# uberkk/ImageCompressionLearnedLiftingandLearnedTreeBasedModels

Measured on AMD Instinct MI355X. Metric: Mpixels/sec (lifting DWT + entropy-model fwd) at 512x512 RGB, higher is better.
Workload: dtype f32 storage, f16x3 arithmetic (3 fp16 MFMA products per fp32 MAC, fp32 accumulate)

## Files before the change

### imagecompressionlearnedliftingandlearnedtreebasedmodels_amd/csrc/conv_f16x3.hip

```cpp
#include "common.h"
#include "split_f16.h"
#include "lifting_f16.h"
#include "plc_fold.h"
#include <string.h>
#include <type_traits>

namespace lldwt {

constexpr int F3_CK = 32;
constexpr int F3_TH = 8, F3_TW = 32;
constexpr int F3_IH = F3_TH + 2, F3_IW = F3_TW + 2, F3_NPX = F3_IH * F3_IW;
constexpr int F3_PITCH = F3_CK * 2 + 16;
constexpr int F3_PART = F3_NPX * F3_PITCH;
constexpr int F3_BUF = 2 * F3_PART;
constexpr int F3_LDS = 2 * F3_BUF + 64;
constexpr int F3_OCB = 128;
constexpr int F3_STEP_BYTES = 2048;
constexpr int F3_CHUNK_BYTES = 9 * 2 * F3_STEP_BYTES;
constexpr int F3_HDR = 256;
constexpr int F3_NTASK = F3_NPX * (F3_CK / 8);
constexpr int F3_R = (F3_NTASK + 255) / 256;

constexpr int F1_HDR = 2048;
constexpr int F1_CHUNK_BYTES = 2 * F3_STEP_BYTES;
// ... 113 lines not shown
    for (int o = 32; o > 0; o >>= 1) {
        mw = fmaxf(mw, __shfl_xor(mw, o, 64));
        ml1 = fmaxf(ml1, __shfl_xor(ml1, o, 64));
        mb = fmaxf(mb, __shfl_xor(mb, o, 64));
    }
    if ((tid & 63) == 0) { red[0][tid >> 6] = mw; red[1][tid >> 6] = ml1; red[2][tid >> 6] = mb; }
    __syncthreads();
    const float amw = fmaxf(fmaxf(red[0][0], red[0][1]), fmaxf(red[0][2], red[0][3]));
    const float sw1 = pow2_scale<15>(amw);
    if (tid == 0) {
        hdr[0] = sw1;
        hdr[1] = fmaxf(fmaxf(red[1][0], red[1][1]), fmaxf(red[1][2], red[1][3]));
        hdr[2] = fmaxf(fmaxf(red[2][0], red[2][1]), fmaxf(red[2][2], red[2][3]));
    }
    const int nch = (cmid + F3_CK - 1) / F3_CK;
    for (int i = tid; i < nch * F3_CK; i += 256) hdr[16 + i] = i < cmid ? bp[i] : 0.f;
    _Float16* fr = reinterpret_cast<_Float16*>(pp + F1_HDR);
    for (int i = tid; i < nch * 2 * 512; i += 256) {
        const int j = i & 7, lane = (i >> 3) & 63, ks = (i >> 9) & 1, chunk = i >> 10;
        const int c = chunk * F3_CK + (lane & 31), k = 16 * ks + 8 * (lane >> 5) + j;
        float v = 0.f;
        if (c < cmid && k < 27) v = wp[c * 27 + k] * sw1;
        const _Float16 hi = (_Float16)v;
        fr[(chunk * 2 + ks) * 1024 + lane * 8 + j] = hi;
        fr[(chunk * 2 + ks) * 1024 + 512 + lane * 8 + j] = (_Float16)(v - (float)hi);
        reinterpret_cast<__bf16*>(pp + F1_HDR + (int64_t)nch * F1_CHUNK_BYTES)[(chunk * 2 + ks) * 512 + lane * 8 + j] = (__bf16)v;
    }
    _Float16* f16 = reinterpret_cast<_Float16*>(pp + f1_w16_off(cmid));
    for (int i = tid; i < w3_nch(cmid) * 512; i += 256) {
        const int j = i & 7, lane = (i >> 3) & 63, chunk = i >> 9;
        const int c = chunk * W3_CK + (lane & 15), k = 8 * (lane >> 4) + j;
        float v = 0.f;
        if (c < cmid && k < 27) v = wp[c * 27 + k] * sw1;
        const _Float16 hi = (_Float16)v;
        f16[chunk * 1024 + lane * 8 + j] = hi;
        f16[chunk * 1024 + 512 + lane * 8 + j] = (_Float16)(v - (float)hi);
    }
}

struct F3Args {
    const float* x;
    float* y;
    const uint8_t* packed;
    const float* bias;
    const float* slots;
    const _Float16* x16;
    const float* xscale;
    const float* parent;
    const uint8_t* packed1;
    int64_t plane_bytes1;
    int cin, cout, act, batch, h, w, tiles_x, nch;
    int64_t plane_bytes;
    unsigned long long* stamps;
};
#define F3_STAMP(i)                                                                                                     \
    if (a.stamps && lane == 0)                                                                                          \
        a.stamps[((((int64_t)blockIdx.z * gridDim.y + blockIdx.y) * gridDim.x + blockIdx.x) * 4 + wave) * 16 + (i)] =   \
            (i) >= 14 ? __builtin_amdgcn_s_memrealtime() : __builtin_amdgcn_s_memtime();

template <int MODE, int PREC = 0, bool S16 = false>
__global__ __launch_bounds__(256) __attribute__((amdgpu_waves_per_eu(1, 1))) void k_conv3_f16x3(F3Args a) {
    constexpr bool IN16 = MODE == 1, FUSED = MODE == 2;
    static_assert(PREC == 0 || FUSED, "the one-product modes exist for the fused pair (eval path)");
    constexpr int SB = PREC == 2 ? F3_STEP_BYTES / 2 : F3_STEP_BYTES;
    extern __shared__ __attribute__((aligned(16))) uint8_t lds[];
    const int tid = threadIdx.x, lane = tid & 63, wave = tid >> 6;
    const int64_t z = blockIdx.z;
    const int plane = (int)(z / a.batch);
    const int ocb = blockIdx.y;
    const int ty = blockIdx.x / a.tiles_x, tx = blockIdx.x - ty * a.tiles_x;
    const int y0 = ty * F3_TH, x0 = tx * F3_TW;
    const int h = a.h, w = a.w;
    const int64_t hw = (int64_t)h * w;

    F3_STAMP(0)
    F3_STAMP(14)
    float sx = 1.f;
    if constexpr (IN16) {
        sx = a.xscale[plane];
    } else if constexpr (FUSED) {
    } else {
        float amax = a.slots[plane * 64 + lane];
#pragma unroll
        for (int o = 32; o > 0; o >>= 1) amax = fmaxf(amax, __shfl_xor(amax, o, 64));
        sx = pow2_scale<15>(amax);
    }
    const uint8_t* pp = a.packed + (int64_t)plane * a.plane_bytes;
    const float sw = *reinterpret_cast<const float*>(pp);
    float out_scale = (1.f / sx) * (1.f / sw);

    unsigned pix[F3_R];
    int icg8[F3_R];
    int woff[F3_R];
    bool inimg[F3_R];
#pragma unroll
    for (int r = 0; r < F3_R; ++r) {
        const int task = tid + r * 256;
        const bool live = task < F3_NTASK;
        const int icg = live ? task / F3_NPX : 0, p = live ? task - icg * F3_NPX : 0;
        const int ly = p / F3_IW, lx = p - ly * F3_IW;
        const int gy = y0 - 1 + ly, gx = x0 - 1 + lx;
        const bool in = live && gy >= 0 && gy < h && gx >= 0 && gx < w;
        inimg[r] = in;
        icg8[r] = icg * 8;
        woff[r] = p * F3_PITCH + icg * 16;
        pix[r] = in ? (IN16 ? 2u : 4u) * (unsigned)(gy * w + gx) : 0u;
// ... 545 lines not shown
__device__ __forceinline__ void wino_u(const float* g, double (&u)[4]) {
    const double g0 = g[0], g1 = g[1], g2 = g[2];
    u[0] = g0; u[1] = (g0 + g1 + g2) * 0.5; u[2] = (g0 - g1 + g2) * 0.5; u[3] = g2;
}

__global__ void k_f3w_umax(const float* __restrict__ w, int64_t nrows, uint8_t* __restrict__ packed, int64_t plane_bytes, int64_t woff) {
    const int plane = blockIdx.y;
    float m = 0.f;
    for (int64_t i = blockIdx.x * (int64_t)blockDim.x + threadIdx.x; i < nrows; i += (int64_t)gridDim.x * blockDim.x) {
        double u[4];
        wino_u(w + ((int64_t)plane * nrows + i) * 3, u);
        for (int k = 0; k < 4; ++k) m = fmaxf(m, fabsf((float)u[k]));
    }
#pragma unroll
    for (int o = 32; o > 0; o >>= 1) m = fmaxf(m, __shfl_down(m, o, 64));
    float* hdr = reinterpret_cast<float*>(packed + (int64_t)plane * plane_bytes + woff);
    if ((threadIdx.x & 63) == 0 && m > 0.f) atomicMax(reinterpret_cast<int*>(hdr + 1), __float_as_int(m));
}

__global__ void k_f3w_pack(const float* __restrict__ w, uint8_t* __restrict__ packed, int cin, int cout, int64_t plane_bytes, int64_t woff) {
    const int plane = blockIdx.y;
    uint8_t* pp = packed + (int64_t)plane * plane_bytes + woff;
    float* hdr = reinterpret_cast<float*>(pp);
    const double su = pow2_scale<15>(hdr[1]);
    const int nch = w3_nch(cin), nocb = (cout + F3_OCB - 1) / F3_OCB;
    const int64_t n = (int64_t)nocb * 4 * nch * W3_NST * 64 * 8;
    const float* wp = w + (int64_t)plane * cout * cin * 9;
    _Float16* out = reinterpret_cast<_Float16*>(pp + F3_HDR);
    for (int64_t i = blockIdx.x * (int64_t)blockDim.x + threadIdx.x; i < n; i += (int64_t)gridDim.x * blockDim.x) {
        int64_t r = i;
        const int j = (int)(r % 8); r /= 8;
        const int lane = (int)(r % 64); r /= 64;
        const int st = (int)(r % W3_NST); r /= W3_NST;
        const int chunk = (int)(r % nch); r /= nch;
        const int wv = (int)(r % 4); r /= 4;
        const int ocb = (int)r;
        const int oc = ocb * F3_OCB + wv * 32 + (lane & 31), ic = chunk * W3_CK + 8 * (lane >> 5) + j;
        const int dy = st >> 2, xi = st & 3;
        float v = 0.f;
        if (oc < cout && ic < cin) {
            double u[4];
            wino_u(wp + ((int64_t)oc * cin + ic) * 9 + dy * 3, u);
            v = (float)(u[xi] * su);
        }
        const _Float16 hi = (_Float16)v;
        const int64_t step = ((int64_t)(ocb * 4 + wv) * nch + chunk) * W3_NST + st;
        out[step * 1024 + lane * 8 + j] = hi;
        out[step * 1024 + 512 + lane * 8 + j] = (_Float16)(v - (float)hi);
    }
    if (blockIdx.x == 0 && threadIdx.x == 0) hdr[0] = (float)su;
}

template <bool EARLIER>
__global__ __launch_bounds__(256) __attribute__((amdgpu_waves_per_eu(1, 1))) void k_plc_wino(F3Args a) {
    extern __shared__ __attribute__((aligned(16))) uint8_t lds[];
    const int tid = threadIdx.x, lane = tid & 63, wave = tid >> 6;
    const int64_t z = blockIdx.z;
    const int plane = (int)(z / a.batch);
    const int nocb = (a.cout + F3_OCB - 1) / F3_OCB;
    const int npass = (!EARLIER && gridDim.y == 1) ? nocb : 1;
    int ocb = blockIdx.y;
#define W3_STAMP(i)                                                                                                     \
    if (a.stamps && lane == 0)                                                                                          \
        a.stamps[((((int64_t)blockIdx.z * nocb + ocb) * gridDim.x + blockIdx.x) * 4 + wave) * 16 + (i)] =               \
            (i) >= 14 ? __builtin_amdgcn_s_memrealtime() : __builtin_amdgcn_s_memtime();
    const int ty = blockIdx.x / a.tiles_x, tx = blockIdx.x - ty * a.tiles_x;
    const int y0 = ty * F3_TH, x0 = tx * F3_TW;
    const int h = a.h, w = a.w;
    const int64_t hw = (int64_t)h * w;

    W3_STAMP(0)
    W3_STAMP(14)
    const uint8_t* pp = a.packed + (int64_t)plane * a.plane_bytes + f3_wino_off(a.cin, a.cout);
    const float su = *reinterpret_cast<const float*>(pp);
    const uint8_t* pk1 = a.packed1 + (int64_t)plane * a.plane_bytes1;
    const float* h1 = reinterpret_cast<const float*>(pk1);
    const float* bias1 = h1 + 16;
    const int hp = h >> 1, wp_ = w >> 1;
    const float* par = a.parent + z * 3 * (int64_t)hp * wp_;
    static_assert(F1_PP <= 512, "two patch values per thread");
    float pv[2] = {0.f, 0.f};
    if constexpr (!EARLIER) {
#pragma unroll
        for (int k = 0; k < 2; ++k) {
            const int i = min(tid + 256 * k, F1_PP - 1);
            const int ci = i / 108, rem = i - ci * 108, r = rem / 18, c = rem - r * 18;
            const int Yp = (y0 >> 1) - 1 + r, Xp = (x0 >> 1) - 1 + c;
            pv[k] = par[(int64_t)ci * hp * wp_ + min(max(Yp, 0), hp - 1) * wp_ + min(max(Xp, 0), wp_ - 1)];
        }
    }
    const uint8_t* wbase = pp + F3_HDR + ((int64_t)(ocb * 4 + wave) * a.nch) * (W3_NST * F3_STEP_BYTES) + lane * 16;
    half8 ah[W3_RING], al[W3_RING];
#pragma unroll
    for (int i = 0; i < W3_RING - 1; ++i) {
        ah[i] = *reinterpret_cast<const half8*>(wbase + i * F3_STEP_BYTES);
        al[i] = *reinterpret_cast<const half8*>(wbase + i * F3_STEP_BYTES + 1024);
    }
    half8 w1h, w1l;
    f4_t b1r, b1v;
#define W3_FUSED_LOAD(C1)                                                                                             \
    {                                                                                                                 \
        const uint8_t* w1_ = pk1 + f1_w16_off(a.cin) + (int64_t)((C1) / W3_CK) * F3_STEP_BYTES + lane * 16;           \
        w1h = *reinterpret_cast<const half8*>(w1_);                                                                   \
        w1l = *reinterpret_cast<const half8*>(w1_ + 1024);                                                            \
        b1r = *reinterpret_cast<const f4_t*>(bias1 + (C1) + 4 * (lane >> 4));                                        \
    }
    W3_FUSED_LOAD(0)
    float bias2 = 0.f, bias2n = 0.f;
#define W3_BIAS_LOAD(DST, OCB)                                                                                        \
    {                                                                                                                 \
        const int oc_ = (OCB) * F3_OCB + tid;                                                                         \
        if (tid < F3_OCB && a.bias && oc_ < a.cout) DST = a.bias[plane * a.cout + oc_];                               \
    }
    if constexpr (!EARLIER) {
        W3_BIAS_LOAD(bias2, ocb)
        if (npass > 1) W3_BIAS_LOAD(bias2n, ocb + 1)
    }

    float* PP = reinterpret_cast<float*>(lds + W3_PP);
    float amax = 0.f;
#pragma unroll
    for (int i = tid; i < F1_PP; i += 256) {
        const int ci = i / 108, rem = i - ci * 108, r = rem / 18, c = rem - r * 18;
        const int Yp = (y0 >> 1) - 1 + r, Xp = (x0 >> 1) - 1 + c;
        const bool in = Yp >= 0 && Yp < hp && Xp >= 0 && Xp < wp_;
        const float v = EARLIER ? par[(int64_t)ci * hp * wp_ + min(max(Yp, 0), hp - 1) * wp_ + min(max(Xp, 0), wp_ - 1)] : pv[i >> 8];
        const float vz = in ? v : 0.f;
        PP[i] = vz;
        amax = fmaxf(amax, fabsf(vz));
    }
#pragma unroll
    for (int o = 32; o > 0; o >>= 1) amax = fmaxf(amax, __shfl_xor(amax, o, 64));
    float* red = reinterpret_cast<float*>(lds + W3_DUMP + 32);
    if (lane == 0) red[wave] = amax;
    __syncthreads();
    amax = fmaxf(fmaxf(red[0], red[1]), fmaxf(red[2], red[3]));
    const float s_p = pow2_scale<15>(amax);
    const float sx = 0.5f * pow2_scale<15>(amax * h1[1] + h1[2]);
    const float out_scale = (1.f / sx) * (1.f / su);
    const float inv1sx = (1.f / s_p) * (1.f / h1[0]) * sx;
    W3_STAMP(12)
    if constexpr (EARLIER) {
    for (int px = tid; px < F3_NPX; px += 256) {
        const int ly = px / F3_IW, lx = px - ly * F3_IW;
        uint8_t* dst = lds + W3_COL + ((lx & 1) * (F3_IH * 17) + ly * 17 + (lx >> 1)) * W3_COLP;
#pragma unroll
        for (int g = 0; g < 4; ++g) {
            float v8[8];
#pragma unroll
            for (int j = 0; j < 8; ++j) {
                const int k = 8 * g + j, q = k < 27 ? k : 26;
                const int dy = (q % 9) / 3, dx = q % 3;
                v8[j] = PP[(q / 9) * 108 + ((ly + dy) >> 1) * 18 + ((lx + dx) >> 1)] * s_p;
            }
            half8 ch_, cl_;
            split8v(v8, ch_, cl_);
            *reinterpret_cast<half8*>(dst + g * 16) = ch_;
            *reinterpret_cast<half8*>(dst + 64 + g * 16) = cl_;
        }
    }
    } else {
        switch (__builtin_amdgcn_readfirstlane(wave)) {
            case 0: w3_im2col_group<0>(lds, PP, s_p, lane); break;
            case 1: w3_im2col_group<1>(lds, PP, s_p, lane); break;
            case 2: w3_im2col_group<2>(lds, PP, s_p, lane); break;
            default: w3_im2col_group<3>(lds, PP, s_p, lane); break;
        }
    }

    const int p = lane & 15, g = lane >> 4;
    int colw[3], vw[3];
    unsigned pinm = 0;
// ... 5 lines not shown
        const int rr = live ? r : 0;
        colw[B] = W3_COL + (rr * 17 + p) * W3_COLP + g * 16;
        vw[B] = live ? ((rr * 4) * 16 + p) * 32 + (((g >> 1) ^ (p >> 3)) * 16) + (g & 1) * 8 : -1;
        const int gy = y0 - 1 + r;
#pragma unroll
        for (int s = 0; s < 4; ++s) {
            const int gx = x0 - 1 + 2 * p + s;
            pin[B][s] = live && gy >= 0 && gy < h && gx >= 0 && gx < w;
            if (pin[B][s]) pinm |= 1u << (4 * B + s);
        }
    }
    const int en = p < 6 ? p : 0, er = wave + 4 * (en >> 1);
    const bool elive = p < 6 && er < F3_IH;
    const int cole = W3_COL + (((en & 1) * F3_IH + (elive ? er : 0)) * 17 + 16) * W3_COLP + g * 16;
    const int pine = (elive && y0 - 1 + er >= 0 && y0 - 1 + er < h && x0 + 31 + (en & 1) < w) ? -1 : 0;
    half8 c1h[4], c1l[4];
    f4_t t1[4];
    float d1[4][4];
#define W3_ROW_READ(B)                                                                                                \
    {                                                                                                                 \
        _Pragma("unroll") for (int s = 0; s < 4; ++s) {                                                               \
            const uint8_t* c_ = lds + colw[B] + ((s & 1) * (F3_IH * 17) + (s >> 1)) * W3_COLP;                        \
            c1h[s] = *reinterpret_cast<const half8*>(c_);                                                             \
            c1l[s] = *reinterpret_cast<const half8*>(c_ + 64);                                                        \
        }                                                                                                             \
    }
#define W3_ROW_MMA() w3_row_mma(t1, w1h, w1l, c1h, c1l);
#define W3_ROW_ACT(B)                                                                                                 \
    {                                                                                                                 \
        if ((B) == 0) b1v = b1r * sx;                                                                                 \
        _Pragma("unroll") for (int s = 0; s < 4; ++s)                                                                 \
            _Pragma("unroll") for (int q = 0; q < 4; ++q) {                                                           \
                const float v_ = __builtin_fmaf(t1[s][q], inv1sx, b1v[q]);                                            \
                d1[s][q] = (pinm >> (4 * (B) + s)) & 1 ? fmaxf(v_, 0.01f * v_) : 0.f;                                 \
            }                                                                                                         \
    }
#define W3_ROW_STORE(B, DST)                                                                                          \
    {                                                                                                                 \
        const bool livev_ = vw[B] >= 0;                                                                               \
        uint8_t* d0_ = livev_ ? (DST) + vw[B] : lds + W3_DUMP;                                                        \
        const int xs_ = livev_ ? 16 * 32 : 0, lo_ = livev_ ? W3_PART : 8;                                             \
        _Pragma("unroll") for (int xi = 0; xi < 4; ++xi) {                                                            \
            float v4_[4];                                                                                             \
            _Pragma("unroll") for (int q = 0; q < 4; ++q)                                                             \
                v4_[q] = xi == 0 ? d1[0][q] - d1[2][q] : xi == 1 ? d1[1][q] + d1[2][q]                                \
                       : xi == 2 ? d1[2][q] - d1[1][q] : d1[1][q] - d1[3][q];                                         \
            h4_t hi_, lo4_;                                                                                           \
            split4v(v4_, hi_, lo4_);                                                                                  \
            *reinterpret_cast<h4_t*>(d0_ + xi * xs_) = hi_;                                                           \
            *reinterpret_cast<h4_t*>(d0_ + xi * xs_ + lo_) = lo4_;                                                    \
        }                                                                                                             \
    }
    if constexpr (!EARLIER) {
        if (tid < F3_OCB) reinterpret_cast<float*>(lds + W3_BIAS)[tid] = bias2;
        if (npass > 1 && tid < F3_OCB) reinterpret_cast<float*>(lds + W3_BIAS)[F3_OCB + tid] = bias2n;
    }
    half8 c2h[3][2], c2l[3][2], ceh, cel;
    f4_t t2[3][2], te;
    float d2[3][4][4], de[4];
#define W3_ROW_READ2(B)                                                                                               \
    {                                                                                                                 \
        _Pragma("unroll") for (int s = 0; s < 2; ++s) {                                                               \
            const uint8_t* c_ = lds + colw[B] + s * (F3_IH * 17) * W3_COLP;                                           \
            c2h[B][s] = *reinterpret_cast<const half8*>(c_);                                                          \
            c2l[B][s] = *reinterpret_cast<const half8*>(c_ + 64);                                                     \
        }                                                                                                             \
    }
#define W3_ROW_MMA2(B) w3_row_mma2(t2[B][0], t2[B][1], w1h, w1l, c2h[B][0], c2h[B][1], c2l[B][0], c2l[B][1]);
#define W3_ROW_MMA3() w3_row_mma3(t2[0][0], t2[0][1], te, w1h, w1l, c2h[0][0], c2h[0][1], ceh, c2l[0][0], c2l[0][1], cel);
#define W3_ROW_ACT2(B, S)                                                                                             \
    {                                                                                                                 \
        _Pragma("unroll") for (int q = 0; q < 4; ++q) {                                                               \
            const float v_ = __builtin_fmaf(t2[B][S][q], inv1sx, b1v[q]);                                             \
            d2[B][S][q] = pin[B][S] ? fmaxf(v_, 0.01f * v_) : 0.f;                                                    \
        }                                                                                                             \
    }
#define W3_EXTRA_ACT()                                                                                                \
    {                                                                                                                 \
        b1v = b1r * sx;                                                                                               \
        _Pragma("unroll") for (int q = 0; q < 4; ++q) {                                                               \
            const float v_ = __builtin_fmaf(te[q], inv1sx, b1v[q]);                                                   \
            de[q] = __int_as_float(__float_as_int(fmaxf(v_, 0.01f * v_)) & pine);                                     \
        }                                                                                                             \
    }
#define W3_ROW_SHIFT(B)                                                                                               \
    {                                                                                                                 \
        _Pragma("unroll") for (int q = 0; q < 4; ++q) {                                                               \
            d2[B][2][q] = w3_dpp<0x101, false>(w3_dpp<0x110 + 15 - 2 * (B), true>(0.f, de[q]), d2[B][0][q]);          \
            d2[B][3][q] = w3_dpp<0x101, false>(w3_dpp<0x110 + 14 - 2 * (B), true>(0.f, de[q]), d2[B][1][q]);          \
        }                                                                                                             \
    }
#define W3_ROW_STORE2(B, DST, XI)                                                                                     \
    {                                                                                                                 \
        const bool livev_ = vw[B] >= 0;                                                                               \
        uint8_t* d0_ = livev_ ? (DST) + vw[B] : lds + W3_DUMP;                                                        \
        const int xs_ = livev_ ? 16 * 32 : 0, lo_ = livev_ ? W3_PART : 8;                                             \
        float v4_[4];                                                                                                 \
        _Pragma("unroll") for (int q = 0; q < 4; ++q)                                                                 \
            v4_[q] = (XI) == 0 ? d2[B][0][q] - d2[B][2][q] : (XI) == 1 ? d2[B][1][q] + d2[B][2][q]                    \
                   : (XI) == 2 ? d2[B][2][q] - d2[B][1][q] : d2[B][1][q] - d2[B][3][q];                               \
        h4_t hi_, lo4_;                                                                                               \
        w3_split4(v4_, hi_, lo4_);                                                                                    \
        *reinterpret_cast<h4_t*>(d0_ + (XI) * xs_) = hi_;                                                             \
        *reinterpret_cast<h4_t*>(d0_ + (XI) * xs_ + lo_) = lo4_;                                                      \
    }
    W3_STAMP(13)
    __syncthreads();
    W3_STAMP(2)

    floatx16 acc[4][4];
#define W3_ZERO_ACC()                                                                                                 \
    _Pragma("unroll") for (int xi = 0; xi < 4; ++xi)                                                                  \
        _Pragma("unroll") for (int n = 0; n < 4; ++n)                                                                 \
            _Pragma("unroll") for (int q = 0; q < 16; ++q) acc[xi][n][q] = 0.f;
    if constexpr (EARLIER) {
        W3_ZERO_ACC()
#pragma unroll
        for (int B = 0; B < 3; ++B) {
            W3_ROW_READ(B)
            W3_ROW_MMA()
            W3_ROW_ACT(B)
            W3_ROW_STORE(B, lds)
        }
    } else {
        ceh = *reinterpret_cast<const half8*>(lds + cole);
        cel = *reinterpret_cast<const half8*>(lds + cole + 64);
        W3_ROW_READ2(0) W3_ROW_READ2(1) W3_ROW_READ2(2)
        W3_ROW_MMA3() W3_ROW_MMA2(1) W3_ROW_MMA2(2)
        W3_EXTRA_ACT()
        W3_FUSED_LOAD((a.nch > 1 ? 1 : 0) * W3_CK)
        W3_ROW_ACT2(0, 0) W3_ROW_ACT2(0, 1) W3_ROW_SHIFT(0)
        W3_ROW_STORE2(0, lds, 0) W3_ROW_STORE2(0, lds, 1) W3_ROW_STORE2(0, lds, 2) W3_ROW_STORE2(0, lds, 3)
        W3_ROW_ACT2(1, 0) W3_ROW_ACT2(1, 1) W3_ROW_SHIFT(1)
        W3_ROW_STORE2(1, lds, 0) W3_ROW_STORE2(1, lds, 1) W3_ROW_STORE2(1, lds, 2) W3_ROW_STORE2(1, lds, 3)
        W3_ROW_ACT2(2, 0) W3_ROW_ACT2(2, 1) W3_ROW_SHIFT(2)
        W3_ROW_STORE2(2, lds, 0) W3_ROW_STORE2(2, lds, 1) W3_ROW_STORE2(2, lds, 2) W3_ROW_STORE2(2, lds, 3)
    }
    if constexpr (EARLIER) __syncthreads();

    const int boff = (((lane >> 4) & 1) * 64 + p) * 32 + (((lane >> 5) ^ (p >> 3)) * 16);
    half8 bh[2][4], bl[2][4];
#define W3_BLOAD_AT(BB, U, SET)                                                                        \
        {                                                                                              \
            const int dy_ = (U) >> 2, xi_ = (U) & 3;                                                   \
            _Pragma("unroll") for (int n = 0; n < 4; ++n) {                                            \
                const int off = ((2 * n + dy_) * 4 + xi_) * 512;                                       \
                bh[SET][n] = *reinterpret_cast<const half8*>((BB) + off);                              \
                bl[SET][n] = *reinterpret_cast<const half8*>((BB) + W3_PART + off);                    \
            }                                                                                          \
        }
#pragma nounroll
    for (int pass = 0; pass < npass; ++pass) {
    const bool succ = !EARLIER && pass + 1 < npass;
    if constexpr (!EARLIER) {
        if (pass > 0) {
            W3_STAMP(0)
            W3_STAMP(14)
            W3_STAMP(12)
            W3_STAMP(13)
            W3_STAMP(2)
            wbase += (int64_t)4 * a.nch * (W3_NST * F3_STEP_BYTES);
            bias2n = 0.f;
            if (succ) W3_BIAS_LOAD(bias2n, ocb + 1)
            W3_BLOAD_AT(lds + ((pass * a.nch) & 1) * W3_BUF + boff, 0, 0)
            ceh = *reinterpret_cast<const half8*>(lds + cole);
            cel = *reinterpret_cast<const half8*>(lds + cole + 64);
        }
        W3_ZERO_ACC()
        if (pass == 0) {
            __syncthreads();
            W3_BLOAD_AT(lds + boff, 0, 0)
        }
    }
    W3_STAMP(1)
    for (int chunk = 0; chunk < a.nch; ++chunk) {
        if (chunk >= 2 && chunk < 16 && !(chunk & 1)) W3_STAMP(2 + (chunk >> 1))
        const int buf = EARLIER ? chunk & 1 : (pass * a.nch + chunk) & 1;
        const uint8_t* wp = wbase + (int64_t)chunk * (W3_NST * F3_STEP_BYTES);
        const uint8_t* wpn = wp + (succ && chunk + 1 == a.nch ? (int64_t)3 * a.nch * (W3_NST * F3_STEP_BYTES) : 0);
        const uint8_t* bb = lds + buf * W3_BUF + boff;
        uint8_t* sdst = lds + (buf ^ 1) * W3_BUF;
        const int c1 = (chunk + 1 < a.nch ? chunk + 1 : succ ? 0 : chunk) * W3_CK;
        int n2 = chunk + 2;
        if (n2 >= a.nch) {
            n2 = succ ? n2 - a.nch : a.nch - 1;
            if (n2 >= a.nch) n2 -= a.nch;
        }
        const int c2 = n2 * W3_CK;
#define W3_BLOAD(U, SET) W3_BLOAD_AT(bb, U, SET)
        if constexpr (EARLIER) {
            W3_BLOAD(0, 0)
            __builtin_amdgcn_sched_barrier(0);
        }
#pragma unroll
        for (int u = 0; u < W3_NST; ++u) {
            const int xi = u & 3;
            const uint8_t* wr = u + W3_RING - 1 < W3_NST ? wp : wpn;
            ah[(u + W3_RING - 1) % W3_RING] = *reinterpret_cast<const half8*>(wr + (u + W3_RING - 1) * F3_STEP_BYTES);
            al[(u + W3_RING - 1) % W3_RING] = *reinterpret_cast<const half8*>(wr + (u + W3_RING - 1) * F3_STEP_BYTES + 1024);
            if (u + 1 < W3_NST) W3_BLOAD(u + 1, (u + 1) & 1)
            if constexpr (EARLIER) {
                if (u == 0) W3_FUSED_LOAD(c1)
                if (u == 2 || u == 5 || u == 8) W3_ROW_READ((u - 2) / 3)
                if (u == 3 || u == 6 || u == 9) W3_ROW_MMA()
                if (u == 4 || u == 7 || u == 10) W3_ROW_ACT((u - 4) / 3)
                if (u == 5 || u == 8 || u == 11) W3_ROW_STORE((u - 5) / 3, sdst)
            } else {
                if (u == W3_NST - 1) W3_BLOAD_AT(sdst + boff, 0, 0)
                if (u == 0) W3_ROW_READ2(0)
                if (u == 1) { W3_ROW_MMA3() W3_ROW_READ2(1) }
                if (u == 2) { W3_EXTRA_ACT() W3_ROW_ACT2(0, 0) W3_ROW_ACT2(0, 1) W3_ROW_MMA2(1) W3_ROW_READ2(2) }
                if (u == 3) { W3_ROW_SHIFT(0) W3_ROW_STORE2(0, sdst, 0) W3_ROW_STORE2(0, sdst, 1) }
                if (u == 4) { W3_ROW_STORE2(0, sdst, 2) W3_ROW_STORE2(0, sdst, 3) W3_ROW_ACT2(1, 0) W3_ROW_MMA2(2) }
                if (u == 5) { W3_ROW_ACT2(1, 1) W3_ROW_SHIFT(1) W3_ROW_STORE2(1, sdst, 0) }
                if (u == 6) { W3_ROW_STORE2(1, sdst, 1) W3_ROW_STORE2(1, sdst, 2) W3_ROW_ACT2(2, 0) }
                if (u == 7) { W3_ROW_STORE2(1, sdst, 3) W3_ROW_ACT2(2, 1) W3_ROW_SHIFT(2) }
                if (u == 8) { W3_ROW_STORE2(2, sdst, 0) W3_ROW_STORE2(2, sdst, 1) W3_FUSED_LOAD(c2) }
                if (u == 9) W3_ROW_STORE2(2, sdst, 2)
                if (u == 10) W3_ROW_STORE2(2, sdst, 3)
            }
            const half8 A_h = ah[u % W3_RING], A_l = al[u % W3_RING];
#pragma unroll
            for (int n = 0; n < 4; ++n) acc[xi][n] = mma32<0>(A_l, bh[u & 1][n], acc[xi][n]);
#pragma unroll
            for (int n = 0; n < 4; ++n) acc[xi][n] = mma32<0>(A_h, bl[u & 1][n], acc[xi][n]);
#pragma unroll
            for (int n = 0; n < 4; ++n) acc[xi][n] = mma32<0>(A_h, bh[u & 1][n], acc[xi][n]);
#pragma unroll
            for (int i = 0; i < 12; ++i) {
                __builtin_amdgcn_sched_group_barrier(0x008, 1, 0);
                __builtin_amdgcn_sched_group_barrier(0x100, 1, 0);
                __builtin_amdgcn_sched_group_barrier(0x020, 1, 0);
                if constexpr (EARLIER) __builtin_amdgcn_sched_group_barrier(0x002, 8, 0);
                else if (i >= 8) __builtin_amdgcn_sched_group_barrier(0x002, 6, 0);
                else __builtin_amdgcn_sched_group_barrier(0x002, 4, 0);
                __builtin_amdgcn_sched_group_barrier(0x200, 1, 0);
            }
            __builtin_amdgcn_sched_barrier(0);
            if constexpr (!EARLIER) {
                if (u == W3_NST - 2) __syncthreads();
            }
        }
#undef W3_BLOAD
        if constexpr (EARLIER) __syncthreads();
    }
#undef W3_BLOAD_AT
#undef W3_ROW_READ
#undef W3_ROW_MMA
#undef W3_ROW_ACT
#undef W3_ROW_STORE
#undef W3_ROW_READ2
#undef W3_ROW_MMA2
#undef W3_ROW_MMA3
#undef W3_ROW_ACT2
#undef W3_EXTRA_ACT
#undef W3_ROW_SHIFT
#undef W3_ROW_STORE2

    W3_STAMP(10)
    if constexpr (!EARLIER) {
        if (succ && pass > 0 && tid < F3_OCB) reinterpret_cast<float*>(lds + W3_BIAS)[((pass + 1) & 1) * F3_OCB + tid] = bias2n;
    }
    int eh = h, ew = w, ey0 = y0, ex0 = x0, elane = lane;
    if constexpr (!EARLIER) asm volatile("" : "+s"(eh), "+s"(ew), "+s"(ey0), "+s"(ex0), "+v"(elane));
    const int64_t ehw = (int64_t)eh * ew;
    const int ep = elane & 15;
    const int ocw = ocb * F3_OCB + __builtin_amdgcn_readfirstlane(wave) * 32;
    const int och = 4 * (elane >> 5), orow = (elane >> 4) & 1;
    float* ybase = a.y + (z * a.cout + ocw) * ehw + (int64_t)ey0 * ew;
    const unsigned loff = (unsigned)och * (unsigned)ehw + (unsigned)(orow * ew + ex0 + 2 * ep);
    const bool full = ey0 + F3_TH <= eh && ex0 + F3_TW <= ew;
    if constexpr (EARLIER) {
#define W3_EPI(COND, ACT0, ACT1)                                                                                      \
    _Pragma("unroll") for (int q = 0; q < 16; ++q) {                                                                  \
        const int ocq = (q & 3) + 8 * (q >> 2);                                                                       \
        if (ocw + ocq + och < a.cout) {                                                                               \
            const float bq = a.bias ? a.bias[plane * a.cout + ocw + ocq + och] : 0.f;                                 \
            float* yq = ybase + (int64_t)ocq * ehw + loff;                                                            \
            _Pragma("unroll") for (int n = 0; n < 4; ++n) {                                                           \
                const float v0 = (acc[0][n][q] + acc[1][n][q] + acc[2][n][q]) * out_scale + bq;                       \
                const float v1 = (acc[1][n][q] - acc[2][n][q] - acc[3][n][q]) * out_scale + bq;                       \
                if (COND) *reinterpret_cast<f2_t*>(yq + 2 * n * ew) = f2_t{ACT0, ACT1};                               \
            }                                                                                                         \
        }                                                                                                             \
    }
    if (full && a.act != LLDWT_ACT_TANH) {
        const float slope = a.act == LLDWT_ACT_LRELU ? 0.01f : (a.act == LLDWT_ACT_RELU ? 0.f : 1.f);
        W3_EPI(true, fmaxf(v0, v0 * slope), fmaxf(v1, v1 * slope))
    } else {
        const bool colin = ex0 + 2 * ep < ew;
        W3_EPI(colin && ey0 + 2 * n + orow < eh, act_apply(v0, a.act), act_apply(v1, a.act))
    }
#undef W3_EPI
    } else {
    float bq[16];
    {
        const f4_t* bl = reinterpret_cast<const f4_t*>(lds + W3_BIAS +
                                                       ((pass & 1) * F3_OCB + __builtin_amdgcn_readfirstlane(wave) * 32 + och) * 4);
#pragma unroll
        for (int k = 0; k < 4; ++k) {
            const f4_t b4 = bl[2 * k];
#pragma unroll
            for (int j = 0; j < 4; ++j) bq[4 * k + j] = b4[j];
        }
    }
    asm volatile("s_nop 7\n\ts_nop 7\n\ts_nop 4");
#define W3_EPI(COND, ACT0, ACT1)                                                                                      \
    float os_ = out_scale;                                                                                            \
    asm volatile("" : "+v"(os_));                                                                                     \
    _Pragma("unroll") for (int q = 0; q < 16; ++q) {                                                                  \
        const int ocq = (q & 3) + 8 * (q >> 2);                                                                       \
        if (ocw + ocq + och < a.cout) {                                                                               \
            float* yq = ybase + (int64_t)ocq * ehw + loff;                                                            \
            _Pragma("unroll") for (int n = 0; n < 4; ++n) {                                                           \
                const float m0 = w3_acc_read(acc[0][n][q]), m1 = w3_acc_read(acc[1][n][q]);                           \
                const float m2 = w3_acc_read(acc[2][n][q]), m3 = w3_acc_read(acc[3][n][q]);                           \
                const float v0 = (m0 + m1 + m2) * os_ + bq[q];                                                        \
                const float v1 = (m1 - m2 - m3) * os_ + bq[q];                                                        \
                if (COND) *reinterpret_cast<f2_t*>(yq + 2 * n * ew) = f2_t{ACT0, ACT1};                               \
            }                                                                                                         \
        }                                                                                                             \
    }
    if (full && a.act != LLDWT_ACT_TANH) {
        const float slope = a.act == LLDWT_ACT_LRELU ? 0.01f : (a.act == LLDWT_ACT_RELU ? 0.f : 1.f);
        { W3_EPI(true, fmaxf(v0, v0 * slope), fmaxf(v1, v1 * slope)) }
    } else {
        const bool colin = ex0 + 2 * ep < ew;
#define W3_IN (colin && ey0 + 2 * n + orow < eh)
        if (a.act == LLDWT_ACT_TANH) {
            { W3_EPI(W3_IN, fast_tanh(v0), fast_tanh(v1)) }
        } else if (a.act == LLDWT_ACT_LRELU) {
            { W3_EPI(W3_IN, v0 >= 0.f ? v0 : 0.01f * v0, v1 >= 0.f ? v1 : 0.01f * v1) }
        } else if (a.act == LLDWT_ACT_RELU) {
            { W3_EPI(W3_IN, v0 > 0.f ? v0 : 0.f, v1 > 0.f ? v1 : 0.f) }
        } else {
            { W3_EPI(W3_IN, v0, v1) }
        }
#undef W3_IN
    }
#undef W3_EPI
    }
    W3_STAMP(11)
    W3_STAMP(15)
    ++ocb;
    }
#undef W3_FUSED_LOAD
#undef W3_BIAS_LOAD
#undef W3_ZERO_ACC
#undef W3_STAMP
}
#undef F3_STAMP

}
using namespace lldwt;

static const int g_f3_shape16 = [] { const char* e = getenv("LLDWT_PLC_SHAPE"); return (e && !strcmp(e, "16")) ? 1 : 0; }();
static int f3_shape16() { return g_f3_shape16; }
extern "C" int lldwt_plc_shape16(void) { return g_f3_shape16; }

static const int g_plc_wino = [] { const char* e = getenv("LLDWT_PLC_ALGO"); return (e && !strcmp(e, "direct")) ? 0 : 1; }();
static bool plc_wino_active() { return g_plc_wino && !g_f3_shape16; }
extern "C" int lldwt_plc_winograd(void) { return plc_wino_active() ? 1 : 0; }

extern "C" int64_t lldwt_conv_f16x3_packed_bytes(int cin, int cout) {
    if (cin <= 0 || cout <= 0) return -1;
    return f3_plane_bytes(cin, cout);
}

extern "C" int lldwt_conv_f16x3_pack(const float* w, void* packed, int cin, int cout, int64_t planes, void* stream) {
    LLDWT_REQUIRE(w && packed && cin > 0 && cout > 0 && planes > 0 && planes <= 65535, "conv_f16x3_pack: bad arguments");
    hipStream_t st = (hipStream_t)stream;
    const int64_t pb = f3_plane_bytes(cin, cout);
    for (int64_t p = 0; p < planes; ++p)
        if (hipMemsetAsync(reinterpret_cast<char*>(packed) + p * pb, 0, F3_HDR, st) != hipSuccess) {
            set_error("conv_f16x3_pack: memset failed");
            return LLDWT_EHIP;
        }
    const int64_t nw = (int64_t)cout * cin * 9;
    hipLaunchKernelGGL(k_f3_wmax, dim3(64, (unsigned)planes), dim3(256), 0, st, w, nw, reinterpret_cast<float*>(packed), pb);
    hipLaunchKernelGGL(k_f3_pack, dim3(1024, (unsigned)planes), dim3(256), 0, st, w, reinterpret_cast<uint8_t*>(packed), cin, cout, pb,
                       f3_shape16());
    if (plc_wino_active()) {
        const int64_t wo = f3_wino_off(cin, cout);
        for (int64_t p = 0; p < planes; ++p)
            if (hipMemsetAsync(reinterpret_cast<char*>(packed) + p * pb + wo, 0, F3_HDR, st) != hipSuccess) {
                set_error("conv_f16x3_pack: memset failed");
                return LLDWT_EHIP;
            }
        hipLaunchKernelGGL(k_f3w_umax, dim3(64, (unsigned)planes), dim3(256), 0, st, w, (int64_t)cout * cin * 3,
                           reinterpret_cast<uint8_t*>(packed), pb, wo);
        hipLaunchKernelGGL(k_f3w_pack, dim3(1024, (unsigned)planes), dim3(256), 0, st, w, reinterpret_cast<uint8_t*>(packed), cin, cout,
                           pb, wo);
    }
    return check_launch("conv_f16x3_pack");
}

extern "C" int lldwt_absmax_slots(const float* x, int64_t planes, int64_t n_per_plane, float* slots, void* stream) {
    LLDWT_REQUIRE(x && slots && planes > 0 && planes <= 65535 && n_per_plane > 0, "absmax_slots: bad arguments");
    const int vec = (((uintptr_t)x) & 15) == 0 && (n_per_plane & 3) == 0;
    hipStream_t st = (hipStream_t)stream;
// ... 52 lines not shown
    a.x16 = reinterpret_cast<const _Float16*>(x16); a.xscale = xscale;
    a.parent = nullptr; a.packed1 = nullptr; a.plane_bytes1 = 0; a.stamps = nullptr;
    a.cin = cin; a.cout = cout; a.act = act; a.batch = (int)batch; a.h = (int)h; a.w = (int)w_;
    a.tiles_x = (int)cdiv(w_, F3_TW);
    a.nch = f3_nch(cin);
    a.plane_bytes = f3_plane_bytes(cin, cout);
    const int tiles_y = (int)cdiv(h, F3_TH);
    static bool attr_set = false;
    if (!attr_set) {
        if (hipFuncSetAttribute((const void*)k_conv3_f16x3<1>, hipFuncAttributeMaxDynamicSharedMemorySize, F3_LDS) != hipSuccess ||
            hipFuncSetAttribute((const void*)k_conv3_f16x3<1, 0, true>, hipFuncAttributeMaxDynamicSharedMemorySize, F3_LDS) != hipSuccess) {
            set_error("conv3x3_f16in: cannot reserve %d bytes of LDS", F3_LDS);
            return LLDWT_EHIP;
        }
        attr_set = true;
    }
    dim3 grid((unsigned)(a.tiles_x * tiles_y), (unsigned)f3_nocb(cout), (unsigned)(planes * batch));
    if (g_f3_shape16) hipLaunchKernelGGL((k_conv3_f16x3<1, 0, true>), grid, dim3(256), F3_LDS, (hipStream_t)stream, a);
    else hipLaunchKernelGGL(k_conv3_f16x3<1>, grid, dim3(256), F3_LDS, (hipStream_t)stream, a);
    return check_launch("conv3x3_f16in");
}


extern "C" int64_t lldwt_plc_fused_pack1_bytes(int cmid) { return cmid > 0 && cmid <= 256 ? f1_plane_bytes(cmid) : -1; }

extern "C" int lldwt_plc_fused_pack1(const float* w1, const float* b1, void* packed1, int cmid, int64_t planes, void* stream) {
    LLDWT_REQUIRE(w1 && b1 && packed1 && cmid > 0 && cmid <= 256 && planes > 0 && planes <= 65535, "plc_fused_pack1: bad arguments");
    hipLaunchKernelGGL(k_f1_pack, dim3((unsigned)planes), dim3(256), 0, (hipStream_t)stream, w1, b1,
                       reinterpret_cast<uint8_t*>(packed1), cmid, f1_plane_bytes(cmid));
    return check_launch("plc_fused_pack1");
}

static unsigned long long* g_f3_stamps = nullptr;
static int64_t g_f3_stamps_bytes = 0;
namespace lldwt { void f3_set_stamps(void* p, int64_t nbytes) { g_f3_stamps = reinterpret_cast<unsigned long long*>(p); g_f3_stamps_bytes = p ? nbytes : 0; } }
static int g_f3_flags = 0;
namespace lldwt { void f3_set_debug(int flags) { g_f3_flags = flags; } }

extern "C" int lldwt_plc_fused(const float* parent, float* y, const void* packed1, const void* packed2, const float* bias2,
                               int cmid, int cout, int act, int64_t planes, int64_t batch, int64_t h, int64_t w_, void* stream) {
    LLDWT_REQUIRE(parent && y && packed1 && packed2, "plc_fused: null pointer");
    LLDWT_REQUIRE(cmid > 0 && cmid <= 256 && cout > 0 && planes > 0 && batch > 0 && h > 0 && w_ > 0 && planes * batch <= 65535,
                  "plc_fused: bad dims");
    LLDWT_REQUIRE(h % 2 == 0 && w_ % 2 == 0, "plc_fused: the output is the 2x-upsampled parent's size: even h, w");
    LLDWT_REQUIRE(act == LLDWT_ACT_NONE || act == LLDWT_ACT_LRELU || act == LLDWT_ACT_TANH || act == LLDWT_ACT_RELU, "plc_fused: bad activation");
    F3Args a;
    a.x = nullptr; a.y = y; a.packed = reinterpret_cast<const uint8_t*>(packed2); a.bias = bias2; a.slots = nullptr;
    a.x16 = nullptr; a.xscale = nullptr;
    a.parent = parent; a.packed1 = reinterpret_cast<const uint8_t*>(packed1); a.plane_bytes1 = f1_plane_bytes(cmid);
    a.cin = cmid; a.cout = cout; a.act = act; a.batch = (int)batch; a.h = (int)h; a.w = (int)w_;
    a.tiles_x = (int)cdiv(w_, F3_TW);
    a.nch = f3_nch(cmid);
    a.plane_bytes = f3_plane_bytes(cmid, cout);
    const int tiles_y = (int)cdiv(h, F3_TH);
    {
        const int64_t need = (int64_t)a.tiles_x * tiles_y * f3_nocb(cout) * planes * batch * 4 * 16 * 8;
        a.stamps = (g_f3_stamps && g_f3_stamps_bytes >= need) ? g_f3_stamps : nullptr;
    }
    static bool attr_set = false;
    if (!attr_set) {
        if (hipFuncSetAttribute((const void*)k_conv3_f16x3<2, 0>, hipFuncAttributeMaxDynamicSharedMemorySize, F1_LDS) != hipSuccess ||
            hipFuncSetAttribute((const void*)k_conv3_f16x3<2, 1>, hipFuncAttributeMaxDynamicSharedMemorySize, F1_LDS) != hipSuccess ||
            hipFuncSetAttribute((const void*)k_conv3_f16x3<2, 2>, hipFuncAttributeMaxDynamicSharedMemorySize, F1_LDS) != hipSuccess ||
            hipFuncSetAttribute((const void*)k_conv3_f16x3<2, 0, true>, hipFuncAttributeMaxDynamicSharedMemorySize, F1_LDS) != hipSuccess ||
            hipFuncSetAttribute((const void*)k_conv3_f16x3<2, 1, true>, hipFuncAttributeMaxDynamicSharedMemorySize, F1_LDS) != hipSuccess ||
            hipFuncSetAttribute((const void*)k_conv3_f16x3<2, 2, true>, hipFuncAttributeMaxDynamicSharedMemorySize, F1_LDS) != hipSuccess) {
            set_error("plc_fused: cannot reserve %d bytes of LDS", F1_LDS);
            return LLDWT_EHIP;
        }
        attr_set = true;
    }
    dim3 grid((unsigned)(a.tiles_x * tiles_y), (unsigned)f3_nocb(cout), (unsigned)(planes * batch));
    const int prec = split_precision();
    if (prec == 0 && plc_wino_active()) {
        static bool wattr_set = false;
        if (!wattr_set) {
            if (hipFuncSetAttribute((const void*)k_plc_wino<false>, hipFuncAttributeMaxDynamicSharedMemorySize, W3_LDS) != hipSuccess ||
                hipFuncSetAttribute((const void*)k_plc_wino<true>, hipFuncAttributeMaxDynamicSharedMemorySize, W3_LDS_EARLIER) != hipSuccess) {
                set_error("plc_fused: cannot reserve %d bytes of LDS", W3_LDS);
                return LLDWT_EHIP;
            }
            wattr_set = true;
        }
        a.nch = w3_nch(cmid);
        if (g_f3_flags & 1) hipLaunchKernelGGL(k_plc_wino<true>, grid, dim3(256), W3_LDS_EARLIER, (hipStream_t)stream, a);
        else {
            static const int cus = [] {
                int dev = 0, n = 0;
                if (hipGetDevice(&dev) != hipSuccess || hipDeviceGetAttribute(&n, hipDeviceAttributeMultiprocessorCount, dev) != hipSuccess) n = 0;
                return n;
            }();
            const bool fold = (g_f3_flags & 2) ? false : (g_f3_flags & 4) ? true : plc_fold_pays((int64_t)grid.x * grid.z, cus, (int)grid.y);
            if (fold) grid.y = 1;
            hipLaunchKernelGGL(k_plc_wino<false>, grid, dim3(256), W3_LDS, (hipStream_t)stream, a);
        }
    } else if (g_f3_shape16) {
        if (prec == 1) hipLaunchKernelGGL((k_conv3_f16x3<2, 1, true>), grid, dim3(256), F1_LDS, (hipStream_t)stream, a);
        else if (prec == 2) hipLaunchKernelGGL((k_conv3_f16x3<2, 2, true>), grid, dim3(256), F1_LDS, (hipStream_t)stream, a);
        else hipLaunchKernelGGL((k_conv3_f16x3<2, 0, true>), grid, dim3(256), F1_LDS, (hipStream_t)stream, a);
    } else if (prec == 1) hipLaunchKernelGGL((k_conv3_f16x3<2, 1>), grid, dim3(256), F1_LDS, (hipStream_t)stream, a);
    else if (prec == 2) hipLaunchKernelGGL((k_conv3_f16x3<2, 2>), grid, dim3(256), F1_LDS, (hipStream_t)stream, a);
    else hipLaunchKernelGGL((k_conv3_f16x3<2, 0>), grid, dim3(256), F1_LDS, (hipStream_t)stream, a);
    return check_launch("plc_fused");
}
```

Baseline: 213.8.

## Make Winograd PLC kernel persistent with grid-stride units and prefetched parent patch

Converts the non-EARLIER k_plc_wino launch into a persistent kernel with one block per CU by default. Each block loops over (plane, ocb, tile) work units with stride equal to the resident count. The parent-patch load for the next unit is issued before the current unit's pass loop, so its latency overlaps compute. Bias loads become unconditional clamped loads, with the masking moved to the LDS store. The aim is to remove block launch and tail overhead and hide the patch fetch latency, at the cost of extra register pressure and possible load imbalance when units do not divide evenly by CUs.

```diff
diff --git a/imagecompressionlearnedliftingandlearnedtreebasedmodels_amd/csrc/conv_f16x3.hip b/imagecompressionlearnedliftingandlearnedtreebasedmodels_amd/csrc/conv_f16x3.hip
--- a/imagecompressionlearnedliftingandlearnedtreebasedmodels_amd/csrc/conv_f16x3.hip
+++ b/imagecompressionlearnedliftingandlearnedtreebasedmodels_amd/csrc/conv_f16x3.hip
@@ -189,6 +189,7 @@
     int cin, cout, act, batch, h, w, tiles_x, nch;
     int64_t plane_bytes;
     unsigned long long* stamps;
+    int tiles, units, fold, resident;
 };
 #define F3_STAMP(i)                                                                                                     \
     if (a.stamps && lane == 0)                                                                                          \
@@ -840,22 +841,76 @@
 }
 
 template <bool EARLIER>
-__global__ __launch_bounds__(256) __attribute__((amdgpu_waves_per_eu(1, 1))) void k_plc_wino(F3Args a) {
+__global__ __launch_bounds__(256) __attribute__((amdgpu_waves_per_eu(1, 1))) void k_plc_wino(F3Args a0) {
     extern __shared__ __attribute__((aligned(16))) uint8_t lds[];
-    const int tid = threadIdx.x, lane = tid & 63, wave = tid >> 6;
-    const int64_t z = blockIdx.z;
+    static_assert(F1_PP <= 512, "two patch values per thread");
+#define W3_PATCH_LOAD(A, DST, U)                                                                                      \
+    {                                                                                                                 \
+        const int nt_ = A.tiles, hp_ = A.h >> 1, wq_ = A.w >> 1;                                                      \
+        const int u_ = min((U), A.units - 1), q_ = u_ / nt_, t_ = u_ - q_ * nt_;                                      \
+        const int z_ = A.fold ? q_ : q_ / ((A.cout + F3_OCB - 1) / F3_OCB);                                           \
+        const int ty_ = t_ / A.tiles_x, tx_ = t_ - ty_ * A.tiles_x;                                                   \
+        const float* par_ = A.parent + (int64_t)z_ * 3 * ((int64_t)hp_ * wq_);                                        \
+        _Pragma("unroll") for (int k = 0; k < 2; ++k) {                                                               \
+            const int i = min(tid + 256 * k, F1_PP - 1);                                                              \
+            const int ci = i / 108, rem = i - ci * 108, r = rem / 18, c = rem - r * 18;                               \
+            const int Yp = ty_ * (F3_TH >> 1) - 1 + r, Xp = tx_ * (F3_TW >> 1) - 1 + c;                               \
+            DST[k] = par_[(int64_t)ci * hp_ * wq_ + min(max(Yp, 0), hp_ - 1) * wq_ + min(max(Xp, 0), wq_ - 1)];       \
+        }                                                                                                             \
+    }
+    float pv[2] = {0.f, 0.f};
+    if constexpr (!EARLIER) {
+        const int tid = threadIdx.x;
+        W3_PATCH_LOAD(a0, pv, (int)blockIdx.x)
+        asm volatile("" : "+v"(pv[0]), "+v"(pv[1]));
+    }
+    int unit_ = blockIdx.x;
+    bool more;
+    const __attribute__((address_space(4))) F3Args* ka_ =
+        (const __attribute__((address_space(4))) F3Args*)__builtin_amdgcn_kernarg_segment_ptr();
+    unsigned klo_ = (unsigned)(uint64_t)ka_, khi_ = (unsigned)((uint64_t)ka_ >> 32);
+#pragma nounroll
+    do {
+    int tid_ = threadIdx.x;
+    if constexpr (!EARLIER) {
+        asm volatile("" : "+v"(tid_), "+v"(klo_), "+v"(khi_), "+v"(unit_));
+        __builtin_assume(tid_ >= 0 && tid_ < 256);
+        klo_ = __builtin_amdgcn_readfirstlane(klo_);
+        khi_ = __builtin_amdgcn_readfirstlane(khi_);
+        ka_ = (const __attribute__((address_space(4))) F3Args*)(((uint64_t)khi_ << 32) | klo_);
+    }
+    const __attribute__((address_space(4))) F3Args& a = *ka_;
+    const int unit = EARLIER ? 0 : __builtin_amdgcn_readfirstlane(unit_);
+    int more_ = !EARLIER && unit + a.resident < a.units;
+    if constexpr (!EARLIER) {
+        unit_ += a.resident;
+        asm volatile("" : "+v"(more_));
+    }
+    const int tid = tid_, lane = tid & 63, wave = tid >> 6;
+    const int nocb = (a.cout + F3_OCB - 1) / F3_OCB;
+    const int npass = (!EARLIER && a.fold) ? nocb : 1;
+    if constexpr (!EARLIER) __builtin_assume(a.cout > 0 && a.nch > 0);
+    const int ntiles = EARLIER ? (int)gridDim.x : a.tiles;
+    const int h = a.h, w = a.w;
+    const int64_t hw = (int64_t)h * w;
+    const int hp = h >> 1, wp_ = w >> 1;
+    int64_t z;
+    int tile, ocb;
+    if constexpr (EARLIER) {
+        z = blockIdx.z; tile = blockIdx.x; ocb = blockIdx.y;
+    } else {
+        const int q = unit / ntiles;
+        tile = unit - q * ntiles;
+        z = a.fold ? q : q / nocb;
+        ocb = a.fold ? 0 : q - (int)z * nocb;
+    }
     const int plane = (int)(z / a.batch);
-    const int nocb = (a.cout + F3_OCB - 1) / F3_OCB;
-    const int npass = (!EARLIER && gridDim.y == 1) ? nocb : 1;
-    int ocb = blockIdx.y;
 #define W3_STAMP(i)                                                                                                     \
     if (a.stamps && lane == 0)                                                                                          \
-        a.stamps[((((int64_t)blockIdx.z * nocb + ocb) * gridDim.x + blockIdx.x) * 4 + wave) * 16 + (i)] =               \
+        a.stamps[(((z * nocb + ocb) * ntiles + tile) * 4 + wave) * 16 + (i)] =                                          \
             (i) >= 14 ? __builtin_amdgcn_s_memrealtime() : __builtin_amdgcn_s_memtime();
-    const int ty = blockIdx.x / a.tiles_x, tx = blockIdx.x - ty * a.tiles_x;
+    const int ty = tile / a.tiles_x, tx = tile - ty * a.tiles_x;
     const int y0 = ty * F3_TH, x0 = tx * F3_TW;
-    const int h = a.h, w = a.w;
-    const int64_t hw = (int64_t)h * w;
 
     W3_STAMP(0)
     W3_STAMP(14)
@@ -864,19 +919,7 @@
     const uint8_t* pk1 = a.packed1 + (int64_t)plane * a.plane_bytes1;
     const float* h1 = reinterpret_cast<const float*>(pk1);
     const float* bias1 = h1 + 16;
-    const int hp = h >> 1, wp_ = w >> 1;
     const float* par = a.parent + z * 3 * (int64_t)hp * wp_;
-    static_assert(F1_PP <= 512, "two patch values per thread");
-    float pv[2] = {0.f, 0.f};
-    if constexpr (!EARLIER) {
-#pragma unroll
-        for (int k = 0; k < 2; ++k) {
-            const int i = min(tid + 256 * k, F1_PP - 1);
-            const int ci = i / 108, rem = i - ci * 108, r = rem / 18, c = rem - r * 18;
-            const int Yp = (y0 >> 1) - 1 + r, Xp = (x0 >> 1) - 1 + c;
-            pv[k] = par[(int64_t)ci * hp * wp_ + min(max(Yp, 0), hp - 1) * wp_ + min(max(Xp, 0), wp_ - 1)];
-        }
-    }
     const uint8_t* wbase = pp + F3_HDR + ((int64_t)(ocb * 4 + wave) * a.nch) * (W3_NST * F3_STEP_BYTES) + lane * 16;
     half8 ah[W3_RING], al[W3_RING];
 #pragma unroll
@@ -896,16 +939,19 @@
     W3_FUSED_LOAD(0)
     float bias2 = 0.f, bias2n = 0.f;
 #define W3_BIAS_LOAD(DST, OCB)                                                                                        \
-    {                                                                                                                 \
-        const int oc_ = (OCB) * F3_OCB + tid;                                                                         \
-        if (tid < F3_OCB && a.bias && oc_ < a.cout) DST = a.bias[plane * a.cout + oc_];                               \
-    }
+    DST = *(a.bias ? a.bias + (plane * a.cout + min((OCB) * F3_OCB + tid, a.cout - 1)) : par);
+#define W3_BIAS_VALUE(SRC, OCB) ((tid < F3_OCB && a.bias && (OCB) * F3_OCB + tid < a.cout) ? SRC : 0.f)
     if constexpr (!EARLIER) {
         W3_BIAS_LOAD(bias2, ocb)
-        if (npass > 1) W3_BIAS_LOAD(bias2n, ocb + 1)
+        W3_BIAS_LOAD(bias2n, ocb + 1)
     }
 
     float* PP = reinterpret_cast<float*>(lds + W3_PP);
+    if constexpr (!EARLIER) {
+        unsigned po_ = (unsigned)(uintptr_t)(__attribute__((address_space(3))) float*)PP;
+        asm volatile("" : "+v"(po_));
+        PP = (float*)(__attribute__((address_space(3))) float*)(uintptr_t)po_;
+    }
     float amax = 0.f;
 #pragma unroll
     for (int i = tid; i < F1_PP; i += 256) {
@@ -1017,8 +1063,9 @@
         }                                                                                                             \
     }
     if constexpr (!EARLIER) {
-        if (tid < F3_OCB) reinterpret_cast<float*>(lds + W3_BIAS)[tid] = bias2;
-        if (npass > 1 && tid < F3_OCB) reinterpret_cast<float*>(lds + W3_BIAS)[F3_OCB + tid] = bias2n;
+        const float b0_ = W3_BIAS_VALUE(bias2, ocb), b1_ = W3_BIAS_VALUE(bias2n, ocb + 1);
+        if (tid < F3_OCB) reinterpret_cast<float*>(lds + W3_BIAS)[tid] = b0_;
+        if (tid < F3_OCB) reinterpret_cast<float*>(lds + W3_BIAS)[F3_OCB + tid] = b1_;
     }
     half8 c2h[3][2], c2l[3][2], ceh, cel;
     f4_t t2[3][2], te;
@@ -1114,6 +1161,7 @@
                 bl[SET][n] = *reinterpret_cast<const half8*>((BB) + W3_PART + off);                    \
             }                                                                                          \
         }
+    if constexpr (!EARLIER) W3_PATCH_LOAD(a, pv, unit + a.resident)
 #pragma nounroll
     for (int pass = 0; pass < npass; ++pass) {
     const bool succ = !EARLIER && pass + 1 < npass;
@@ -1125,8 +1173,7 @@
             W3_STAMP(13)
             W3_STAMP(2)
             wbase += (int64_t)4 * a.nch * (W3_NST * F3_STEP_BYTES);
-            bias2n = 0.f;
-            if (succ) W3_BIAS_LOAD(bias2n, ocb + 1)
+            W3_BIAS_LOAD(bias2n, ocb + 1)
             W3_BLOAD_AT(lds + ((pass * a.nch) & 1) * W3_BUF + boff, 0, 0)
             ceh = *reinterpret_cast<const half8*>(lds + cole);
             cel = *reinterpret_cast<const half8*>(lds + cole + 64);
@@ -1224,7 +1271,8 @@
 
     W3_STAMP(10)
     if constexpr (!EARLIER) {
-        if (succ && pass > 0 && tid < F3_OCB) reinterpret_cast<float*>(lds + W3_BIAS)[((pass + 1) & 1) * F3_OCB + tid] = bias2n;
+        const float bn_ = W3_BIAS_VALUE(bias2n, ocb + 1);
+        if (succ && pass > 0 && tid < F3_OCB) reinterpret_cast<float*>(lds + W3_BIAS)[((pass + 1) & 1) * F3_OCB + tid] = bn_;
     }
     int eh = h, ew = w, ey0 = y0, ex0 = x0, elane = lane;
     if constexpr (!EARLIER) asm volatile("" : "+s"(eh), "+s"(ew), "+s"(ey0), "+s"(ex0), "+v"(elane));
@@ -1309,8 +1357,12 @@
     W3_STAMP(15)
     ++ocb;
     }
+    more = !EARLIER && __builtin_amdgcn_readfirstlane(more_) != 0;
+    } while (more);
+#undef W3_PATCH_LOAD
 #undef W3_FUSED_LOAD
 #undef W3_BIAS_LOAD
+#undef W3_BIAS_VALUE
 #undef W3_ZERO_ACC
 #undef W3_STAMP
 }
@@ -1469,6 +1521,7 @@
     a.tiles_x = (int)cdiv(w_, F3_TW);
     a.nch = f3_nch(cmid);
     a.plane_bytes = f3_plane_bytes(cmid, cout);
+    a.tiles = 0; a.units = 0; a.fold = 0; a.resident = 0;
     const int tiles_y = (int)cdiv(h, F3_TH);
     {
         const int64_t need = (int64_t)a.tiles_x * tiles_y * f3_nocb(cout) * planes * batch * 4 * 16 * 8;
@@ -1508,8 +1561,13 @@
                 return n;
             }();
             const bool fold = (g_f3_flags & 2) ? false : (g_f3_flags & 4) ? true : plc_fold_pays((int64_t)grid.x * grid.z, cus, (int)grid.y);
-            if (fold) grid.y = 1;
-            hipLaunchKernelGGL(k_plc_wino<false>, grid, dim3(256), W3_LDS, (hipStream_t)stream, a);
+            const int64_t units = (int64_t)grid.x * grid.z * (fold ? 1 : (int64_t)grid.y);
+            LLDWT_REQUIRE(units <= (1 << 30), "plc_fused: too many tiles");
+            const int cap = g_f3_flags >> 8;
+            int64_t resident = (g_f3_flags & 8) ? units : cap > 0 ? cap : cus > 0 ? cus : units;
+            if (resident > units) resident = units;
+            a.tiles = (int)grid.x; a.units = (int)units; a.fold = fold ? 1 : 0; a.resident = (int)resident;
+            hipLaunchKernelGGL(k_plc_wino<false>, dim3((unsigned)resident), dim3(256), W3_LDS, (hipStream_t)stream, a);
         }
     } else if (g_f3_shape16) {
         if (prec == 1) hipLaunchKernelGGL((k_conv3_f16x3<2, 1, true>), grid, dim3(256), F1_LDS, (hipStream_t)stream, a);
```

Measured after the change: 213.2. Within noise of the previous version (-0.3%).
